# Aalto5G/pptk

Measured on AMD Instinct MI355X. Metric: Mpkts/s device-resident (cksum+parse+SipHash), 64B & 1500B; % HBM roofline, higher is better.
Workload: dtype u8

## Files before the change

### pptk_amd/csrc/rx_capi.hip

```cpp
#include <errno.h>
#include <stdlib.h>
#include <string.h>

#include <emmintrin.h>

#include <algorithm>
#include <atomic>
#include <condition_variable>
#include <memory>
#include <functional>
#include <mutex>
#include <new>
#include <thread>
#include <unordered_map>
#include <unordered_set>
#include <vector>

#include "../../include/hashseed.h"
#include "rx_internal.h"

using namespace pptk;

struct PartDesc {
  size_t bytes = 0, base = 0;
// ... 342 lines not shown
static int forced_variant(const pptk_rx_ctx *c) {
  static const long force = env_long("PPTK_RX_VARIANT", -1);
  if (c->forced_variant >= 0) return c->forced_variant;
  return force >= 0 && force < RX_NVARIANTS ? (int)force : -1;
}

static uint64_t resident_blocks(const pptk_rx_ctx *c, int variant);

static int grid_for(const pptk_rx_ctx *c, int variant, uint64_t n, uint32_t tpw = 0) {
  const uint64_t ntiles = (n + 63) / 64;
  const uint64_t want_blocks = (ntiles + kWavesPerBlock - 1) / kWavesPerBlock;
  if (tpw > 0) {
    const uint64_t per_block = (uint64_t)kWavesPerBlock * tpw;
    const uint64_t blocks = (ntiles + per_block - 1) / per_block;
    return (int)std::max<uint64_t>(1, std::min<uint64_t>(want_blocks,
                                                         std::max(blocks, resident_blocks(c, variant))));
  }
  return (int)std::max<uint64_t>(1, std::min<uint64_t>(want_blocks, resident_blocks(c, variant)));
}

static uint64_t resident_blocks(const pptk_rx_ctx *c, int variant) {
  static const long grid_mult = std::max(1l, EXP_KNOB("PPTK_RX_GRID_MULT", 1));
  static const int reserve_knob = (int)std::max(0l, EXP_KNOB("PPTK_RX_RESERVE_CUS", 0));
  const int reserve = std::max(reserve_knob, c->coll_cus);
  const uint64_t ncu = (uint64_t)std::max(1, c->ncu - std::min(reserve, c->ncu - 1));
  static const long bpc_knob = EXP_KNOB("PPTK_RX_BPC", 0);
  const uint64_t bpc = bpc_knob > 0 ? (uint64_t)bpc_knob : (uint64_t)c->bpc[variant];
  return ncu * bpc * (uint64_t)grid_mult;
}

static int plan_grid(const pptk_rx_ctx *c, int variant, uint64_t n, uint32_t tpw, RxKArgs &a);

static uint32_t tiles_per_wave(int variant, bool gather) {
  static const long lane = EXP_KNOB("PPTK_RX_LANE_TPW", 4);
  static const long strm = EXP_KNOB("PPTK_RX_GATHER_TPW", 8);
  static const long jumbo = EXP_KNOB("PPTK_RX_JUMBO_TPW", 0);
  static const long fixed = EXP_KNOB("PPTK_RX_FIXED_TPW", 0);
  if (variant == RX_L4) return (uint32_t)std::max(0l, lane);
  if (!gather) return (uint32_t)std::max(0l, fixed);
  return (uint32_t)std::max(0l, variant == RX_T64S2 ? jumbo : strm);
}

static int plan_grid(const pptk_rx_ctx *c, int variant, uint64_t n, uint32_t tpw, RxKArgs &a) {
  a.tail_block = 0;
  a.tail_tile = 0;
  const int grid = grid_for(c, variant, n, tpw);
  static const long pct = EXP_KNOB("PPTK_RX_TAIL_PCT", 0);
  static const long ttpw = EXP_KNOB("PPTK_RX_TAIL_TPW", 1);
  if (tpw == 0 || pct <= 0 || pct >= 100 || ttpw <= 0) return grid;
  const uint64_t ntiles = (n + 63) / 64;
  const uint64_t t2 = ntiles * (uint64_t)pct / 100, t1 = ntiles - t2;
  const uint64_t w1 = (uint64_t)kWavesPerBlock * tpw, w2 = (uint64_t)kWavesPerBlock * (uint64_t)ttpw;
  const uint64_t b1 = (t1 + w1 - 1) / w1, b2 = (t2 + w2 - 1) / w2;
  if (t2 == 0 || b1 < 2 * resident_blocks(c, variant) || b1 + b2 > 0x7fffffffull) return grid;
  a.tail_block = (uint32_t)b1;
  a.tail_tile = t1;
  return (int)(b1 + b2);
}

static uint64_t gcd64(uint64_t a, uint64_t b) {
  while (b) {
    const uint64_t t = a % b;
    a = b;
    b = t;
  }
  return a;
}

static int check_batch(const pptk_rx_ctx *c, const pptk_rx_dev_batch *b) {
  if (!c || !b) return -EINVAL;
  if (b->n == 0) return 0;
  if (!b->d_frames || (!b->d_recs && !b->d_recs32)) return -EINVAL;
  if (b->n > 0xffffffffull) return -EINVAL;
  if (!b->d_off && b->stride == 0 && b->n > 1) return -EINVAL;
  if (!b->d_len && b->fixed_len > 65535) return -EINVAL;
  return 0;
}

static RxKArgs batch_args(const pptk_rx_ctx *c, const pptk_rx_dev_batch *b) {
  RxKArgs a = c->tmpl;
  a.frames = b->d_frames;
  a.off = b->d_off;
  a.len = b->d_len;
  a.perm = b->d_perm;
  a.stride = b->stride;
  a.fixed_len = b->fixed_len;
  a.n = b->n;
  a.recs = b->d_recs;
  a.recs32 = b->d_recs32;
  a.hash = b->d_hash;
  a.frag = b->d_frag;
  a.key = b->d_key;
  return a;
}

static int auto_variant(const pptk_rx_dev_batch *b, bool *lane_ok_out) {
  uint32_t mmax = 15;
  if (!b->d_off) {
    const uint64_t p = (uint64_t)(uintptr_t)b->d_frames;
    const uint64_t gg = gcd64(b->stride % 16 ? b->stride % 16 : 16, 16);
    mmax = (uint32_t)((p % gg) + 16 - gg);
  }
  const uint32_t maxlen = b->d_len ? (b->max_len ? b->max_len : 65535u) : b->fixed_len;
  const bool lane_ok = !b->d_off && !b->d_len && !b->d_perm && !b->d_frag && mmax == 0 &&
                       b->fixed_len <= 64;
  if (lane_ok_out) *lane_ok_out = lane_ok;
  return lane_ok ? RX_L4 : pick_variant(maxlen + mmax);
}

static uint32_t phase_ticks_for(const pptk_rx_dev_batch *b, int variant, int grid) {
  static const long force = EXP_KNOB("PPTK_RX_PHASE_TICKS", -1);
  if (force >= 0) return (uint32_t)force;
  if (!rx_variant_phased(variant) || b->d_perm || (!b->d_recs && !b->d_recs32)) return 0;
  const uint64_t maxlen = b->d_len ? (b->max_len ? b->max_len : 1518u) : b->fixed_len;
  const uint64_t tile_bytes =
      64 * (b->d_off ? std::max<uint64_t>(64, maxlen / 2)
                     : std::min<uint64_t>(std::max<uint64_t>(b->stride, 64), 1u << 20));
  const uint64_t waves = (uint64_t)grid * kWavesPerBlock;
  const uint64_t ticks = tile_bytes * waves * 3 / 4 / 55000;
  return (uint32_t)std::min<uint64_t>(std::max<uint64_t>(ticks, 100), 1000000);
}

#ifdef PPTK_RX_WAVE_TIMES
static uint64_t *g_wave_times = nullptr;
static int g_wave_count = 0;
extern "C" int pptk_rx_wave_times(uint64_t *host, int max_waves) {
  if (!g_wave_times) return -EINVAL;
  const int n = std::min(max_waves, g_wave_count);
  if (hipDeviceSynchronize() != hipSuccess ||
      hipMemcpy(host, g_wave_times, (size_t)n * 16, hipMemcpyDeviceToHost) != hipSuccess)
    return -EIO;
  return n;
}
#endif

static int launch_batch(pptk_rx_ctx *c, const pptk_rx_dev_batch *b, int variant, void *stream) {
  RxKArgs a = batch_args(c, b);
  a.tune = pick_tune(c, variant, b->d_off || b->d_len || b->d_perm,
                     variant == RX_L4 && lane_coalesced(b->stride, b->fixed_len));
  c->last_variant = variant;
  const bool gather = b->d_off || b->d_len || b->d_perm;
  const int grid = plan_grid(c, variant, b->n, tiles_per_wave(variant, gather), a);
  a.phase_ticks = phase_ticks_for(
      b, variant, (int)std::min<uint64_t>((uint64_t)grid, resident_blocks(c, variant)));
#ifdef PPTK_RX_WAVE_TIMES
  if (!g_wave_times && hipMalloc(&g_wave_times, (size_t)65536 * 16) != hipSuccess) return -ENOMEM;
  if (grid * kWavesPerBlock > 65536) return -EINVAL;
  a.wave_times = g_wave_times;
  g_wave_count = grid * kWavesPerBlock;
#endif
  return hip_err(launch_rx(variant, a, grid, (hipStream_t)stream));
}

int pptk_rx_batch_device(struct pptk_rx_ctx *c, const struct pptk_rx_dev_batch *b,
                         void *stream) {
  int rc = check_batch(c, b);
  if (rc || b->n == 0) return rc;
  DeviceScope dg(c->device);
  if (!dg.ok) return -EIO;
  bool lane_ok = false;
  int variant = auto_variant(b, &lane_ok);
  const int tv = c->tuned[b->d_off || b->d_len || b->d_perm ? 1 : 0][variant];
  if (tv >= 0) variant = tv;
  const int fv = forced_variant(c);
  if (fv >= 0) variant = fv;
  if (variant == RX_L4 && !lane_ok) variant = auto_variant(b, nullptr);
  return launch_batch(c, b, variant, stream);
}

static int autotune_candidates(int variant, bool gather, int cand[8]) {
  int n = 0;
  cand[n++] = variant;
  if (variant == RX_T16S6) {
    cand[n++] = RX_T32S3;
    cand[n++] = RX_T32S3D7;
    cand[n++] = RX_T16S7L;
    if (gather) cand[n++] = RX_M6;
  }
  return n;
}

int pptk_rx_autotune(struct pptk_rx_ctx *c, const struct pptk_rx_dev_batch *b, int reps,
                     void *stream) {
  int rc = check_batch(c, b);
  if (rc || b->n == 0) return rc;
  if (reps < 1 || reps > 100) return -EINVAL;
  DeviceScope dg(c->device);
  if (!dg.ok) return -EIO;
  const int base = auto_variant(b, nullptr);
  const int g = b->d_off || b->d_len || b->d_perm ? 1 : 0;
  int cand[8];
  const int nc = autotune_candidates(base, g == 1, cand);
  hipEvent_t e0 = nullptr, e1 = nullptr;
  if (hipEventCreate(&e0) != hipSuccess || hipEventCreate(&e1) != hipSuccess) {
    (void)hipEventDestroy(e0);
    return -EIO;
  }
  const hipStream_t s = (hipStream_t)stream;
  std::vector<std::vector<float>> ms((size_t)nc);
  for (int r = 0; r < reps + 2 && rc == 0; ++r) {
    for (int k = 0; k < nc && rc == 0; ++k) {
      if (hipEventRecord(e0, s) != hipSuccess) rc = -EIO;
      if (rc == 0) rc = launch_batch(c, b, cand[k], stream);
      if (rc == 0 && (hipEventRecord(e1, s) != hipSuccess ||
                      hipEventSynchronize(e1) != hipSuccess))
        rc = -EIO;
      float t = 0.f;
      if (rc == 0 && r >= 2 && hipEventElapsedTime(&t, e0, e1) == hipSuccess)
        ms[(size_t)k].push_back(t);
    }
  }
  int best = base;
  if (rc == 0 && !ms[0].empty()) {
    std::vector<float> med((size_t)nc, 1e30f);
    for (int k = 0; k < nc; ++k) {
      if (ms[(size_t)k].empty()) continue;
      std::sort(ms[(size_t)k].begin(), ms[(size_t)k].end());
      med[(size_t)k] = ms[(size_t)k][ms[(size_t)k].size() / 2];
    }
    int kb = 0;
    for (int k = 1; k < nc; ++k)
      if (med[(size_t)k] < med[(size_t)kb]) kb = k;
    if (kb != 0 && med[(size_t)kb] < 0.99f * med[0]) best = cand[kb];
  }
  (void)hipEventDestroy(e0);
  (void)hipEventDestroy(e1);
  if (rc == 0) c->tuned[g][base] = best == base ? -1 : best;
  return rc;
}

int pptk_rx_place_buffers(struct pptk_rx_ctx *c, const struct pptk_rx_dev_batch *b,
                          const uint8_t *const *fr, int nf, void *const *rc_, int nr, int reps,
                          int *best_f, int *best_r, float *ms_out, void *stream) {
  if (!c || !b || !fr || !rc_ || !best_f || !best_r || nf < 1 || nf > 16 || nr < 1 ||
      nr > 64 || nf * nr > 256 || reps < 1 || reps > 100)
    return -EINVAL;
  for (int k = 0; k < nf; ++k)
    if (!fr[k]) return -EINVAL;
  for (int k = 0; k < nr; ++k)
    if (!rc_[k]) return -EINVAL;
  pptk_rx_dev_batch t = *b;
  const bool c32 = b->d_recs32 != nullptr;
  t.d_frames = fr[0];
  t.d_recs = c32 ? nullptr : (pptk_rx_rec *)rc_[0];
  t.d_recs32 = c32 ? (pptk_rx_rec32 *)rc_[0] : nullptr;
  int rc = check_batch(c, &t);
  if (rc || b->n == 0) {
    if (rc == 0) *best_f = *best_r = 0;
    return rc;
  }
  DeviceScope dg(c->device);
  if (!dg.ok) return -EIO;
  hipEvent_t e0 = nullptr, e1 = nullptr;
  if (hipEventCreate(&e0) != hipSuccess || hipEventCreate(&e1) != hipSuccess) {
    (void)hipEventDestroy(e0);
    return -EIO;
  }
  const hipStream_t s = (hipStream_t)stream;
  const int np = nf * nr;
  std::vector<std::vector<float>> ms((size_t)np);
  for (int r = 0; r <= reps && rc == 0; ++r) {
    for (int p = 0; p < np && rc == 0; ++p) {
      t.d_frames = fr[p / nr];
      if (c32) t.d_recs32 = (pptk_rx_rec32 *)rc_[p % nr];
      else t.d_recs = (pptk_rx_rec *)rc_[p % nr];
      if (hipEventRecord(e0, s) != hipSuccess) rc = -EIO;
      if (rc == 0) rc = pptk_rx_batch_device(c, &t, stream);
      if (rc == 0 && (hipEventRecord(e1, s) != hipSuccess || hipEventSynchronize(e1) != hipSuccess))
        rc = -EIO;
      float x = 0.f;
      if (rc == 0 && r > 0 && hipEventElapsedTime(&x, e0, e1) == hipSuccess)
        ms[(size_t)p].push_back(x);
    }
  }
  (void)hipEventDestroy(e0);
  (void)hipEventDestroy(e1);
  if (rc) return rc;
  int bp = 0;
  float bm = 1e30f;
  for (int p = 0; p < np; ++p) {
    std::vector<float> &v = ms[(size_t)p];
    std::sort(v.begin(), v.end());
    const float med = v.empty() ? 1e30f : v[v.size() / 2];
    if (ms_out) ms_out[p] = med;
    if (med < bm) {
      bm = med;
      bp = p;
    }
  }
  *best_f = bp / nr;
  *best_r = bp % nr;
  return 0;
}

int pptk_rx_place_records(struct pptk_rx_ctx *c, const struct pptk_rx_dev_batch *b,
                          void *const *cands, int ncand, int reps, int *best, float *ms_out,
                          void *stream) {
  if (!b || !best) return -EINVAL;
  const uint8_t *f0 = b->d_frames;
  int bf = 0;
  return pptk_rx_place_buffers(c, b, &f0, 1, cands, ncand, reps, &bf, best, ms_out, stream);
}

static bool tx_two_pass() {
  static const long v = EXP_KNOB("PPTK_TX_TWO_PASS", 1);
  return v != 0;
}

int pptk_tx_cksum_device(struct pptk_rx_ctx *c, uint8_t *d_frames, const uint64_t *d_off,
                         const uint16_t *d_len, uint64_t stride, uint32_t fixed_len,
                         uint64_t n, uint32_t max_len, void *stream) {
  if (!c || n > 0xffffffffull) return -EINVAL;
  if (n == 0) return 0;
  if (!d_frames || (!d_off && stride == 0 && n > 1) || (!d_len && fixed_len > 65535))
    return -EINVAL;
  DeviceScope dg(c->device);
  if (!dg.ok) return -EIO;
  pptk_rx_dev_batch b;
  memset(&b, 0, sizeof(b));
  b.d_frames = d_frames;
  b.d_off = d_off;
  b.d_len = d_len;
  b.stride = stride;
  b.fixed_len = fixed_len;
  b.max_len = max_len;
  b.n = n;
  uint32_t mmax = 15;
  if (!d_off) {
    const uint64_t p = (uint64_t)(uintptr_t)d_frames;
    const uint64_t gg = gcd64(stride % 16 ? stride % 16 : 16, 16);
    mmax = (uint32_t)((p % gg) + 16 - gg);
  }
  const uint32_t maxlen = d_len ? (max_len ? max_len : 65535u) : fixed_len;
  int variant = pick_variant(maxlen + mmax);
  const bool two_pass = !d_off && tx_two_pass();
  if (two_pass) {
    const int tv = c->tuned[0][variant];
    if (tv >= 0 && tv != RX_L4) variant = tv;
  }
  const int fv = forced_variant(c);
  if (fv >= 0 && fv != RX_L4) variant = fv;
  RxKArgs a = batch_args(c, &b);
  a.frames_w = d_frames;
  c->last_variant = variant;
  a.tune = c->forced_flags >= 0 ? (uint32_t)c->forced_flags & kTuneMask
                                : pick_tune(c, variant, d_off || d_len) &
                                      ~(uint32_t)PPTK_RX_TUNE_NT_LOADS;
  hipStream_t s = (hipStream_t)stream;
  if (two_pass) {
    if (c->forced_flags < 0)
      a.tune = pick_tune(c, variant, false);
    uint64_t *side = c->d_txuser && c->txuser_n >= n ? c->d_txuser : nullptr;
    const bool pooled = side == nullptr;
    if (pooled) {
      hipMemPool_t pool;
      {
        std::lock_guard<std::mutex> g(c->txpool_mu);
        if (!c->txpool) {
          hipMemPoolProps pp;
          memset(&pp, 0, sizeof(pp));
          pp.allocType = hipMemAllocationTypePinned;
          pp.location.type = hipMemLocationTypeDevice;
          pp.location.id = c->device;
          hipMemPool_t np = nullptr;
          if (hipMemPoolCreate(&np, &pp) != hipSuccess) return -ENOMEM;
          uint64_t keep = UINT64_MAX;
          (void)hipMemPoolSetAttribute(np, hipMemPoolAttrReleaseThreshold, &keep);
          c->txpool = np;
        }
        pool = c->txpool;
      }
      if (hipMallocFromPoolAsync((void **)&side, n * 8, pool, s) != hipSuccess)
        return -ENOMEM;
    }
    a.txside = side;
    hipError_t e = launch_rx(variant, a, grid_for(c, variant, n), s);
    if (e == hipSuccess) e = launch_tx_apply(side, d_frames, d_off, stride, n, s);
    if (pooled && hipFreeAsync(side, s) != hipSuccess && e == hipSuccess) e = hipErrorUnknown;
    return hip_err(e);
  }
  return hip_err(launch_rx(variant, a, grid_for(c, variant, n), s));
}

int pptk_tx_set_side_buffer(struct pptk_rx_ctx *c, void *d_side, uint64_t frames) {
  if (!c || (!d_side && frames) || ((uintptr_t)d_side & 7u)) return -EINVAL;
  DeviceScope dg(c->device);
  if (!dg.ok) return -EIO;
  c->d_txuser = (uint64_t *)d_side;
  c->txuser_n = d_side ? frames : 0;
  return 0;
}

int pptk_tx_rewrite_device(struct pptk_rx_ctx *c, uint8_t *d_frames, const uint64_t *d_off,
                           const uint16_t *d_len, uint64_t stride, uint32_t fixed_len,
                           uint64_t n, const struct pptk_rewrite *d_rw, uint64_t rw_count,
                           uint8_t *d_status, void *stream) {
  const bool ok = d_rw && (rw_count == 1 || rw_count == n);
  return hdr_op(c, d_frames, d_off, d_len, stride, fixed_len, n, d_status, ok,
                [&](const HdrBatch &b, int grid) {
                  const RewriteKArgs a = {b, d_rw, rw_count == 1 ? 1u : 0u};
                  return launch_rewrite(a, grid, (hipStream_t)stream);
                });
}

int pptk_tcp_mss_clamp_device(struct pptk_rx_ctx *c, uint8_t *d_frames, const uint64_t *d_off,
                              const uint16_t *d_len, uint64_t stride, uint32_t fixed_len,
                              uint64_t n, uint16_t mss, uint32_t flags, uint8_t *d_status,
                              void *stream) {
  const bool ok = !(flags & ~PPTK_MSS_SYN_ONLY);
  return hdr_op(c, d_frames, d_off, d_len, stride, fixed_len, n, d_status, ok,
                [&](const HdrBatch &b, int grid) {
                  const MssKArgs a = {b, mss, flags};
                  return launch_mss_clamp(a, grid, (hipStream_t)stream);
                });
}

int pptk_tcp_seq_translate_device(struct pptk_rx_ctx *c, uint8_t *d_frames, const uint64_t *d_off,
                                  const uint16_t *d_len, uint64_t stride, uint32_t fixed_len,
                                  uint64_t n, const struct pptk_seqxlate *d_xl, uint64_t xl_count,
                                  const uint32_t *d_idx, uint8_t *d_status, void *stream) {
  const bool ok = d_xl && xl_count != 0 && (d_idx || xl_count == 1 || xl_count == n);
  return hdr_op(c, d_frames, d_off, d_len, stride, fixed_len, n, d_status, ok,
                [&](const HdrBatch &b, int grid) {
                  const SeqKArgs a = {b, d_xl, xl_count, d_idx, !d_idx && xl_count == 1 ? 1u : 0u};
                  return launch_seq_translate(a, grid, (hipStream_t)stream);
                });
}

static const BinBounds &bin_bounds() {
  static const BinBounds bb = [] {
    BinBounds r;
    for (int k = 0; k < kGroups - 1; ++k) r.b[k] = kGroupMaxLen[k];
#ifdef PPTK_RX_EXPERIMENTS
    const char *e = getenv("PPTK_RX_BIN_BOUNDS");
#else
    const char *e = nullptr;
#endif
    if (!e) return r;
    BinBounds t = r;
    for (int k = 0; k < kGroups - 1; ++k) {
      char *end = nullptr;
      const unsigned long v = strtoul(e, &end, 10);
      if (end == e || v > 65535 || (k && v < t.b[k - 1])) return r;
      t.b[k] = (uint32_t)v;
      e = *end == ',' ? end + 1 : end;
    }
    return t;
  }();
  return bb;
}

static bool default_bounds(const BinBounds &bb) {
  for (int k = 0; k < kGroups - 1; ++k)
    if (bb.b[k] != kGroupMaxLen[k]) return false;
  return true;
}

int pptk_rx_batch_device_mixed(struct pptk_rx_ctx *c, const struct pptk_rx_dev_batch *b,
                               uint32_t *d_perm, void *d_scratch, void *stream) {
  int rc = check_batch(c, b);
  if (rc || b->n == 0) return rc;
  if (!b->d_len || !d_scratch) return -EINVAL;
  DeviceScope dg(c->device);
  if (!dg.ok) return -EIO;
  const hipStream_t s = (hipStream_t)stream;
  const BinBounds &bb = bin_bounds();
  const bool dflt = default_bounds(bb);
  if (b->max_len && b->max_len <= bb.b[kGroups - 2]) {
    pptk_rx_dev_batch t = *b;
    t.d_perm = nullptr;
    if ((rc = pptk_rx_batch_device(c, &t, stream)) != 0) return rc;
    return d_perm ? hip_err(launch_iota(d_perm, b->n, s)) : 0;
  }
  uint32_t *perm = d_perm ? d_perm : bin_perm(d_scratch, kBinGrid, b->n);
  BinDesc bd{b->d_off, b->stride, bin_desc_off(d_scratch, kBinGrid),
             bin_desc_len(d_scratch, kBinGrid, b->n)};
  hipError_t e = launch_bin(b->d_len, b->n, perm, d_scratch, s, kBinGrid, bd, bb, true);
  if (e != hipSuccess) return -EIO;
  RxKArgs a = batch_args(c, b);
  a.perm = perm;
  a.off = bd.boff;
  a.len = bd.blen;
  a.by_pos = 1;
  const uint32_t *tab = bin_table(d_scratch, kBinGrid);
  a.plan = tab + kGroups + 1;
  a.off0 = b->d_off;
  a.len0 = b->d_len;
  const uint32_t maxlen = b->max_len ? b->max_len : 65535u;
  const int fv = forced_variant(c);
  for (int g = 0; g < kGroups; ++g) {
    const bool last = g == kGroups - 1 || bb.b[g] >= maxlen;
    if (!last && g > 0 && bb.b[g] == bb.b[g - 1]) continue;
    int variant = fv >= 0 && fv != RX_L4 ? fv
                  : dflt || g == kGroups - 1 ? kGroupVariant[g]
                                             : pick_variant(bb.b[g] + 15);
    if (fv < 0 && c->tuned[1][variant] >= 0 && c->tuned[1][variant] != RX_L4)
      variant = c->tuned[1][variant];
    a.plan_group = (uint32_t)g;
    a.range_lo = tab + g;
    a.range_hi = tab + (last ? kGroups : g + 1);
    a.tune = pick_tune(c, variant, true);
    e = launch_rx(variant, a, grid_for(c, variant, b->n), s);
    if (e != hipSuccess) return -EIO;
    if (last) break;
  }
  return 0;
}

int pptk_rx_set_tuning(struct pptk_rx_ctx *c, int variant, int flags) {
  if (!c || variant < -1 || variant >= RX_NVARIANTS || flags < -1) return -EINVAL;
  if (flags >= 0 && ((uint32_t)flags & ~kTuneMask)) return -EINVAL;
  c->forced_variant = variant;
  const int rx = flags < 0 ? -1 : flags & ~PPTK_RX_TUNE_PERMIT_PASSES;
  c->forced_flags = flags >= 0 && rx == 0 && (flags & PPTK_RX_TUNE_PERMIT_PASSES) ? -1 : rx;
  c->permit_passes = flags >= 0 && (flags & PPTK_RX_TUNE_PERMIT_PASSES);
  return 0;
}

static constexpr int kSePerXcc = 4;

int pptk_rx_stream_split(struct pptk_rx_ctx *c, int coll_cus, void **rx_stream,
                         void **coll_stream) {
  if (!c || coll_cus < 0) return -EINVAL;
  if (coll_cus == 0) {
    if (rx_stream) *rx_stream = nullptr;
    if (coll_stream) *coll_stream = nullptr;
    c->coll_cus = 0;
    return 0;
  }
  if (!rx_stream || !coll_stream) return -EINVAL;
  *rx_stream = *coll_stream = nullptr;
  if (c->split_coll && c->split_cus == coll_cus) {
    *rx_stream = c->split_rx;
    *coll_stream = c->split_coll;
    c->coll_cus = coll_cus;
    return 0;
  }
  if (ctx_comm_slot(c)->load(std::memory_order_acquire) != nullptr) return -EBUSY;
  DeviceScope dg(c->device);
  if (!dg.ok) return -EIO;
  int nxcc = 1;
  if (hipDeviceGetAttribute(&nxcc, hipDeviceAttributeNumberOfXccs, c->device) != hipSuccess ||
      nxcc < 1)
    nxcc = 1;
  if (coll_cus % (nxcc * kSePerXcc) || coll_cus >= c->ncu || c->ncu % nxcc) return -EINVAL;
  std::vector<uint32_t> rx((c->ncu + 31) / 32, 0), coll(rx.size(), 0);
  for (int i = 0; i < c->ncu; ++i) (i >= c->ncu - coll_cus ? coll : rx)[i / 32] |= 1u << (i % 32);
  hipStream_t a = nullptr, b = nullptr;
  if (hipExtStreamCreateWithCUMask(&a, (uint32_t)rx.size(), rx.data()) != hipSuccess) return -EIO;
  if (hipExtStreamCreateWithCUMask(&b, (uint32_t)coll.size(), coll.data()) != hipSuccess) {
    (void)hipStreamDestroy(a);
    return -EIO;
  }
  drop_split_streams(c);
  {
    std::lock_guard<std::mutex> g(g_split_mu);
    g_split_owned[a] = c;
    g_split_owned[b] = c;
    g_split_retired.erase(a);
    g_split_retired.erase(b);
  }
  c->split_rx = a;
  c->split_coll = b;
  c->split_cus = coll_cus;
  *rx_stream = a;
  *coll_stream = b;
  c->coll_cus = coll_cus;
  return 0;
}

int pptk_rx_stream_destroy(void *stream) {
  if (!stream) return -EINVAL;
  const hipStream_t s = (hipStream_t)stream;
  {
    std::lock_guard<std::mutex> g(g_split_mu);
    if (g_split_owned.count(s)) return -EBUSY;
    if (g_split_retired.erase(s)) return 0;
  }
  return hip_err(hipStreamDestroy(s));
}

int pptk_rx_variant_count(void) { return RX_NVARIANTS; }

int pptk_rx_last_variant(const struct pptk_rx_ctx *c) { return c ? c->last_variant : -1; }

size_t pptk_rx_permit_scratch_bytes(uint64_t n, uint32_t hash_size) {
  if (hash_size == 0 || (hash_size & (hash_size - 1)) || n > 0xffffffffull) return 0;
  return permit_scratch_bytes(n, hash_size);
}

static int permit_common(struct pptk_rx_ctx *c, const struct pptk_rx_rec *d_recs,
                         const struct pptk_rx_rec32 *d_recs32, const uint32_t *d_keys,
                         uint64_t n, int family, const uint8_t *d_subject, uint32_t *d_tokens,
                         uint8_t *d_verdict, void *d_scratch, void *stream) {
  if (!c || (family != 4 && family != 6) || n > 0xffffffffull) return -EINVAL;
  if ((family == 4 && !c->opts.iphash_bits4) || (family == 6 && !c->opts.iphash_bits6))
    return -EINVAL;
  const uint32_t hs = c->opts.iphash_size;
  if (hs == 0 || (hs & (hs - 1))) return -EINVAL;
  if (n == 0) return 0;
  if ((!d_recs && !d_recs32 && !d_keys) || !d_tokens || !d_verdict || !d_scratch) return -EINVAL;
  DeviceScope dg(c->device);
  if (!dg.ok) return -EIO;
  PermitArgs a{};
  a.recs = d_recs32 || d_keys ? nullptr : d_recs;
  a.recs32 = d_keys ? nullptr : d_recs32;
  a.keys_in = d_keys;
  a.n = n;
  a.subject = d_subject;
  a.tokens = d_tokens;
  a.verdict = d_verdict;
  a.hash_size = hs;
  a.family = family;
  a.ncu = c->ncu - c->coll_cus;
  a.force_passes =
      c->permit_passes || (env_tune() >= 0 && (env_tune() & PPTK_RX_TUNE_PERMIT_PASSES)) ? 1 : 0;
  return hip_err(launch_permit(a, d_scratch, (hipStream_t)stream));
}

int pptk_rx_permit_status(struct pptk_rx_ctx *c, const void *d_scratch, void *stream) {
  if (!c || !d_scratch) return -EINVAL;
  DeviceScope dg(c->device);
  if (!dg.ok) return -EIO;
  return permit_status(d_scratch, (hipStream_t)stream);
}

int pptk_rx_permit_device(struct pptk_rx_ctx *c, const struct pptk_rx_rec *d_recs,
                          const struct pptk_rx_rec32 *d_recs32, uint64_t n, int family,
                          const uint8_t *d_subject, uint32_t *d_tokens, uint8_t *d_verdict,
                          void *d_scratch, void *stream) {
  if (!d_recs && !d_recs32) return -EINVAL;
  return permit_common(c, d_recs, d_recs32, nullptr, n, family, d_subject, d_tokens, d_verdict,
                       d_scratch, stream);
}

int pptk_rx_permit_keys_device(struct pptk_rx_ctx *c, const uint32_t *d_keys, uint64_t n,
                               int family, const uint8_t *d_subject, uint32_t *d_tokens,
                               uint8_t *d_verdict, void *d_scratch, void *stream) {
  if (!d_keys && n) return -EINVAL;
  return permit_common(c, nullptr, nullptr, d_keys, n, family, d_subject, d_tokens, d_verdict,
                       d_scratch, stream);
}

int pptk_rx_tokens_refill_device(struct pptk_rx_ctx *c, uint32_t *d_tokens, uint32_t start,
                                 uint32_t end, uint32_t add, uint32_t initial_tokens,
                                 void *stream) {
  if (!c || !d_tokens || start > end || end > c->opts.iphash_size) return -EINVAL;
  DeviceScope dg(c->device);
  if (!dg.ok) return -EIO;
  return hip_err(launch_refill(d_tokens, start, end, add, initial_tokens, (hipStream_t)stream));
}

size_t pptk_rx_bin_scratch_bytes(uint64_t n) { return bin_scratch_bytes(n, kBinGrid); }

// ... 464 lines not shown
```

### pptk_amd/csrc/rx_kernel.hip

```cpp
#include "frame_view.h"
#include "rx_internal.h"

#include <type_traits>

namespace pptk {

namespace {

constexpr int WAVE = 64;
constexpr int WPB = kWavesPerBlock;
constexpr int IMG_CHUNKS = 8;
#ifndef PPTK_RX_IMG_STRIDE
#define PPTK_RX_IMG_STRIDE 144
#endif
constexpr int IMG_STRIDE = PPTK_RX_IMG_STRIDE;
#ifndef PPTK_RX_TAIL_LDS
#define PPTK_RX_TAIL_LDS 1
#endif
constexpr bool TAIL_LDS = PPTK_RX_TAIL_LDS;
constexpr int TAIL_OFF = 128;
static_assert(!TAIL_LDS || (IMG_STRIDE >= TAIL_OFF + 16 && IMG_STRIDE % 16 == 0),
              "the parked tail chunk lives past the 128-byte image");

typedef uint64_t u64x2 __attribute__((ext_vector_type(2)));
// ... 496 lines not shown
    r1 = (u32x4){w[4], w[5], w[6], w[7]};
    r2 = (u32x4){w[8], w[9], w[10], w[11]};
    r3 = (u32x4){w[12], w[13], w[14], w[15]};
  }
  if (stage) {
    st[0] = r0; st[1] = r1;
    if (!c32) { st[2] = r2; st[3] = r3; }
  } else {
    GLB_AS u32x4 *dst = (GLB_AS u32x4 *)(c32 ? (GLB_AS uint8_t *)a.recs32 + (uint64_t)idx * 32u
                                             : (GLB_AS uint8_t *)a.recs + (uint64_t)idx * 64u);
    dst[0] = r0; dst[1] = r1;
    if (!c32) { dst[2] = r2; dst[3] = r3; }
  }
}

__device__ __forceinline__ void flush_records(const RxKArgs &a, const LDS_AS uint8_t *wimg, uint64_t tile,
                                              int lane, uint32_t my_idx, bool scatter,
                                              LDS_AS u32x4 *stash = nullptr) {
  const bool c32 = a.recs32 != nullptr;
  __builtin_amdgcn_wave_barrier();
  const LDS_AS u32x4 *st = (const LDS_AS u32x4 *)wimg;
  GLB_AS uint8_t *rbase = c32 ? (GLB_AS uint8_t *)a.recs32 : (GLB_AS uint8_t *)a.recs;
  GLB_AS u32x4 *dst = (GLB_AS u32x4 *)(rbase + tile * (uint64_t)WAVE * (c32 ? 32u : 64u));
  const uint64_t nrec = min((uint64_t)WAVE, a.n - tile * WAVE);
  const int lg = c32 ? 1 : 2;
  int kmax = c32 ? 2 : 4;
  if (kDiag && (a.tune & 128u)) kmax >>= 1;
#pragma unroll
  for (int k = 0; k < 4; ++k) {
    const int e = k * WAVE + lane;
    const int r = e >> lg;
    const int piece = e & ((1 << lg) - 1);
    GLB_AS u32x4 *d = dst + e;
    bool live = (uint64_t)r < nrec;
    if (scatter) {
      const uint32_t ridx = __shfl(my_idx, r & (WAVE - 1));
      live = ridx != 0xffffffffu;
      d = (GLB_AS u32x4 *)(rbase + (uint64_t)ridx * (c32 ? 32u : 64u)) + piece;
    }
    if (live && k < kmax) {
      const u32x4 val = st[r * 5 + piece];
      if (stash) {
        stash[e] = val;
      } else if (a.tune & 64u) {
        GLB_AS uint64_t *d8 = (GLB_AS uint64_t *)d;
        __hip_atomic_store(d8, (uint64_t)val.x | ((uint64_t)val.y << 32), __ATOMIC_RELAXED,
                           __HIP_MEMORY_SCOPE_AGENT);
        __hip_atomic_store(d8 + 1, (uint64_t)val.z | ((uint64_t)val.w << 32), __ATOMIC_RELAXED,
                           __HIP_MEMORY_SCOPE_AGENT);
      } else if (a.tune & 32u) {
        asm volatile("" ::: "memory");
        __builtin_nontemporal_store(val, d);
      } else {
        *d = val;
      }
    }
  }
  if (PPTK_RX_HASH_MODE == 2 && a.hash && !scatter && !a.perm && lane < WAVE / 2) {
    const uint32_t r0 = 2u * (uint32_t)lane;
    if ((uint64_t)r0 < nrec) {
      const uint64_t h0 = *(const LDS_AS uint64_t *)(st + r0 * 5 + 4);
      GLB_AS uint64_t *hd = (GLB_AS uint64_t *)a.hash + tile * (uint64_t)WAVE + r0;
      if ((uint64_t)r0 + 1 < nrec && ((uintptr_t)hd & 15u) == 0) {
        const uint64_t h1 = *(const LDS_AS uint64_t *)(st + (r0 + 1) * 5 + 4);
        const u64x2 v = {h0, h1};
        if (a.tune & 32u)
          __builtin_nontemporal_store(v, (GLB_AS u64x2 *)hd);
        else
          *(GLB_AS u64x2 *)hd = v;
      } else {
        hd[0] = h0;
        if ((uint64_t)r0 + 1 < nrec) hd[1] = *(const LDS_AS uint64_t *)(st + (r0 + 1) * 5 + 4);
      }
    }
  }
  __builtin_amdgcn_wave_barrier();
}

__device__ __forceinline__ uint64_t phase_deadline(uint32_t period) {
  const uint64_t rt = __builtin_amdgcn_s_memrealtime();
  return rt - rt % period + period;
}
__device__ __forceinline__ void flush_stash(const RxKArgs &a, const LDS_AS u32x4 *stash, uint64_t tile,
                                            int lane) {
  const bool c32 = a.recs32 != nullptr;
  GLB_AS uint8_t *rbase = c32 ? (GLB_AS uint8_t *)a.recs32 : (GLB_AS uint8_t *)a.recs;
  GLB_AS u32x4 *dst = (GLB_AS u32x4 *)(rbase + tile * (uint64_t)WAVE * (c32 ? 32u : 64u));
  const uint64_t nrec = min((uint64_t)WAVE, a.n - tile * WAVE);
  const int lg = c32 ? 1 : 2;
  const int kmax = c32 ? 2 : 4;
#pragma unroll
  for (int k = 0; k < 4; ++k) {
    const int e = k * WAVE + lane;
    if (k < kmax && (uint64_t)(e >> lg) < nrec) {
      const u32x4 val = stash[e];
      asm volatile("" ::: "memory");
      __builtin_nontemporal_store(val, dst + e);
    }
  }
}

struct TileRange {
  uint64_t first, step, end;
};
__device__ __forceinline__ TileRange wave_tiles(const RxKArgs &a, uint64_t ntiles, int wv) {
  const uint64_t wid = (uint64_t)blockIdx.x * WPB + wv;
  const uint64_t nwaves = (uint64_t)gridDim.x * WPB;
  if (a.tune & 256u) {
    const uint64_t per = (ntiles + nwaves - 1) / nwaves;
    return {wid * per, 1, min(ntiles, (wid + 1) * per)};
  }
  if (a.tail_block == 0) return {wid, nwaves, ntiles};
  if (blockIdx.x < a.tail_block) return {wid, (uint64_t)a.tail_block * WPB, min(a.tail_tile, ntiles)};
  return {a.tail_tile + (uint64_t)(blockIdx.x - a.tail_block) * WPB + wv,
          (uint64_t)(gridDim.x - a.tail_block) * WPB, ntiles};
}
__device__ __forceinline__ uint64_t pf_tile(const TileRange &r, uint64_t ntiles, uint64_t t) {
  return t < r.end ? t : ntiles;
}

template <int T, int S>
constexpr int min_waves_per_simd() { return S * T >= 32 ? 2 : 4; }
#ifndef PPTK_RX_D1_WAVES
#define PPTK_RX_D1_WAVES 3
#endif
template <int T, int S, int D>
constexpr int min_waves() { return D == 1 && S * T >= 32 ? PPTK_RX_D1_WAVES : min_waves_per_simd<T, S>(); }

__device__ __forceinline__ bool group_range(RxKArgs &a) {
  if (a.range_lo && a.plan && !(*a.plan & 1u)) {
    if (((*a.plan >> 8) & 0xffu) != a.plan_group) return false;
    a.perm = nullptr;
    a.perm_ld = (const uint32_t *)a.zero;
    a.perm_msk = 0u;
    a.off_ld = a.off0 ? a.off0 : (const uint64_t *)a.zero;
    a.off_msk = a.off0 ? ~0u : 0u;
    a.stride_g = a.off0 ? 0u : a.stride;
    a.len_ld = a.len0;
    a.len_msk = ~0u;
    a.by_pos = 0;
  } else if (a.range_lo) {
    const uint32_t lo = *a.range_lo, hi = *a.range_hi;
    a.perm_ld += lo;
    if (a.by_pos) {
      a.off_ld += lo;
      a.len_ld += lo;
    }
    a.n = hi > lo ? hi - lo : 0;
    if (a.n == 0) return false;
  }
  return true;
}

template <int T, int S, int D, int AL, bool NT, bool GATHER>
__global__ __launch_bounds__(WAVE * WPB, (min_waves<T, S, D>())) void rx_kernel(RxKArgs a) {
  if constexpr (GATHER) {
    if (!group_range(a)) return;
  }
  __shared__ __attribute__((aligned(16))) uint8_t lds[WPB * WAVE * IMG_STRIDE];
  constexpr int IMGC = (S * T < IMG_CHUNKS) ? S * T : IMG_CHUNKS;
  constexpr uint32_t ALM = (1u << AL) - 1;
  static_assert(T % (D + 1) == 0, "prefetch ring must wrap at the tile boundary");
  constexpr bool PHASED = S * T >= 32 && T <= 32;
  __shared__ __attribute__((aligned(16))) u32x4 stash_lds[PHASED ? WPB * 4 * WAVE : 1];
  const bool phased = PHASED && a.phase_ticks != 0;
  uint64_t st_tile = ~0ull;
  uint64_t st_deadline = 0;
  constexpr bool UNROLL = T <= 32;
  const int lane = threadIdx.x & (WAVE - 1);
  const int wv = threadIdx.x / WAVE;
  const int g = lane / T, j = lane % T;
  LDS_AS uint8_t *wimg = (LDS_AS uint8_t *)lds + wv * WAVE * IMG_STRIDE;
  LDS_AS u32x4 *stash = (LDS_AS u32x4 *)stash_lds + (PHASED ? wv * 4 * WAVE : 0);
  const uint64_t ntiles = (a.n + WAVE - 1) / WAVE;
  const TileRange tr = wave_tiles(a, ntiles, wv);
  const uint64_t step = tr.step, tend = tr.end;

  uint64_t tile = tr.first;
#ifdef PPTK_RX_WAVE_TIMES
  const uint64_t wid = (uint64_t)blockIdx.x * WPB + wv;
  const uint64_t wt_start = __builtin_amdgcn_s_memrealtime();
#endif
  Desc dc = load_desc<GATHER>(a, pf_tile(tr, ntiles, tile), lane);
  Desc dn = load_desc<GATHER>(a, pf_tile(tr, ntiles, tile + step), lane);
  uint32_t idx2 = desc_idx<GATHER>(a, pf_tile(tr, ntiles, tile + 2 * step), lane);
  Buf<S> b[D + 1];
#pragma unroll
  for (int k = 0; k < D; ++k) {
    b[k] = load_round<T, S, AL, NT>(a, dc, k, g, j);
    __builtin_amdgcn_sched_barrier(0);
  }

  while (tile < tend) {
    uint32_t my_sum = 0;
    const uint32_t idx3 = desc_idx<GATHER>(a, pf_tile(tr, ntiles, tile + 3 * step), lane);
    auto group = [&](const int r0) __attribute__((always_inline)) {
#pragma unroll
      for (int u = 0; u <= D; ++u) {
        const int r = r0 + u;
        {
          const int rr = r + D;
          const Desc &dd = rr < T ? dc : dn;
          b[(u + D) % (D + 1)] = load_round<T, S, AL, NT>(a, dd, rr < T ? rr : rr - T, g, j);
        }
        const Buf<S> &cb = b[u];
        const int q = g * T + r;
        const int m = (int)(cb.pb & ALM);
        const int c_img = m >> 4;
        const int nch = (m + (int)cb.pl + 15) >> 4;
        LDS_AS uint8_t *img = wimg + q * IMG_STRIDE;
#pragma unroll
        for (int s = 0; s < S; ++s) {
          if (s * T < IMGC + (int)(ALM >> 4)) {
            const int ci = s * T + j - c_img;
            if (ci >= 0 && ci < IMGC) {
              if constexpr (IMG_STRIDE % 16 == 0) {
                *(LDS_AS u32x4 *)(img + 16 * ci) = cb.v[s];
              } else {
                LDS_AS uint32_t *w = (LDS_AS uint32_t *)(img + 16 * ci);
                w[0] = cb.v[s].x;
                w[1] = cb.v[s].y;
                w[2] = cb.v[s].z;
                w[3] = cb.v[s].w;
              }
            }
          }
        }
        uint32_t acc = 0;
        const int ts = team_start_of(m & 15);
#pragma unroll
        for (int s = 0; s < S; ++s) {
          const int c = s * T + j;
          acc = sum_chunk_from<!GATHER>(cb.v[s], 16 * c - m, ts, (int)cb.pl, acc);
        }
        if (!UNROLL && nch > S * T) {
          const u32x4 *c0 = (const u32x4 *)(a.frames + (cb.pb - (uint64_t)m));
          for (int c = S * T + j; c < nch; c += T)
            acc = sum_chunk_from<true>(ldc<NT>(c0 + c), 16 * c - m, ts, (int)cb.pl, acc);
        }
        if constexpr (GATHER) {
          if constexpr (TAIL_LDS) {
            if (j == T - 1) *(LDS_AS u32x4 *)(img + TAIL_OFF) = cb.v[S - 1];
          } else {
            const uint32_t corr = tail_past_end(cb.v[S - 1], m, (int)cb.pl, ts);
            acc -= (j == T - 1 && nch <= S * T) ? corr : 0u;
          }
        }
        acc = team_sum<T>(acc);
        if (j == r)
          my_sum = acc;
        if (PHASED && u < D && st_tile != ~0ull && __builtin_amdgcn_s_memrealtime() >= st_deadline) {
          flush_stash(a, stash, st_tile, lane);
          st_tile = ~0ull;
        }
      }
    };
#ifdef PPTK_RX_FULL_UNROLL
#pragma unroll(T <= 16 ? T : 1)
#else
#pragma unroll 1
#endif
    for (int r0 = 0; r0 < T - (D + 1); r0 += D + 1) {
      group(r0);
      if (PHASED && st_tile != ~0ull && __builtin_amdgcn_s_memrealtime() >= st_deadline) {
        flush_stash(a, stash, st_tile, lane);
        st_tile = ~0ull;
      }
    }
    const Desc d2 = desc_fill<GATHER>(a, idx2, pf_tile(tr, ntiles, tile + 2 * step), lane);
    __builtin_amdgcn_sched_barrier(0);
    group(T - (D + 1));

    const bool stage = !(a.tune & 2u);
    const bool scatter = GATHER && a.perm;
    if (dc.idx != 0xffffffffu && !(kDiag && (a.tune & 16u))) {
      const int m = (int)(dc.base & 15);
      const int ma = (int)(dc.base & ALM);
      const int nch = (ma + (int)dc.len + 15) >> 4;
      u32x4 tailc = (u32x4){0u, 0u, 0u, 0u};
      if constexpr (GATHER && TAIL_LDS) {
        const u32x4 t = *(const LDS_AS u32x4 *)(wimg + lane * IMG_STRIDE + TAIL_OFF);
        const bool fits = nch <= S * T;
        tailc = (u32x4){fits ? t.x : 0u, fits ? t.y : 0u, fits ? t.z : 0u, fits ? t.w : 0u};
      }
      if (UNROLL) {
        if (nch > S * T) {
          const u32x4 *c0 = (const u32x4 *)(a.frames + (dc.base - (uint64_t)ma));
          for (int c = S * T; c < nch; ++c)
            my_sum = settle(sum_chunk_from<true>(ldc<NT>(c0 + c), 16 * c - ma, 0, (int)dc.len,
                                                 my_sum));
        }
      }
      const FrameView v = {wimg + lane * IMG_STRIDE, (const GLB_AS uint8_t *)a.frames + dc.base, m,
                           16 * IMGC - m};
      LaneRec o;
      lane_generic(a, v, dc.len, dc.base, my_sum, tailc, o);
      if (a.txside)
        a.txside[dc.idx] = o.tx;
      emit_record(a, o, dc.idx, (LDS_AS u32x4 *)wimg + lane * 5, stage);
    }
    if (stage && !(kDiag && (a.tune & 8u)) && (a.recs || a.recs32)) {
      if (PHASED && phased && !scatter) {
        if (st_tile != ~0ull) flush_stash(a, stash, st_tile, lane);
        flush_records(a, wimg, tile, lane, dc.idx, scatter, stash);
        st_tile = tile;
        st_deadline = phase_deadline(a.phase_ticks);
      } else {
        flush_records(a, wimg, tile, lane, dc.idx, scatter);
      }
    }
    tile += step;
    dc = dn;
    dn = d2;
    idx2 = idx3;
  }
  if (PHASED && st_tile != ~0ull) flush_stash(a, stash, st_tile, lane);
#ifdef PPTK_RX_WAVE_TIMES
  if (a.wave_times && lane == 0) {
    a.wave_times[2 * wid] = wt_start;
    a.wave_times[2 * wid + 1] = __builtin_amdgcn_s_memrealtime();
  }
#endif
}

constexpr int M_S = 6;
#ifndef PPTK_RX_M_D
#define PPTK_RX_M_D 1
#endif
#ifndef PPTK_RX_M_WAVES
#define PPTK_RX_M_WAVES 3
#endif
constexpr int M_D = PPTK_RX_M_D;
constexpr int M_SUM = 128;
static_assert(IMG_STRIDE >= M_SUM + 4, "the team sum lives past the 128-byte image");

struct MSched {
  uint32_t n0, n1, n2, e0, e1, e2;
};

__device__ __forceinline__ uint32_t m_rank(uint64_t mask) {
  return __builtin_amdgcn_mbcnt_hi((uint32_t)(mask >> 32),
                                   __builtin_amdgcn_mbcnt_lo((uint32_t)mask, 0u));
}

constexpr int M_RMAX = 24;
__device__ __forceinline__ MSched m_schedule(const Desc &d, int lane, LDS_AS uint8_t *list) {
  const bool valid = d.idx != 0xffffffffu;
  const uint32_t nch = ((uint32_t)(d.base & 15u) + d.len + 15u) >> 4;
  const uint64_t b0 = __ballot(valid && nch <= 24u);
  const uint64_t b1 = __ballot(valid && nch > 24u && nch <= 48u);
  const uint64_t b2 = __ballot(valid && nch > 48u);
  MSched s;
  s.n0 = (uint32_t)__popcll(b0);
  s.n1 = (uint32_t)__popcll(b1);
  s.n2 = (uint32_t)__popcll(b2);
  s.e0 = (s.n0 + 15u) >> 4;
  s.e1 = s.e0 + ((s.n1 + 7u) >> 3);
  s.e2 = s.e1 + ((s.n2 + 3u) >> 2);
  LDS_AS uint32_t *lw = (LDS_AS uint32_t *)list;
  lw[lane] = 0xffffffffu;
  if (lane < M_RMAX * 4 - WAVE) lw[WAVE + lane] = 0xffffffffu;
  const uint32_t c = nch <= 24u ? 0u : nch <= 48u ? 1u : 2u;
  const uint32_t rho = c == 0u ? m_rank(b0) : c == 1u ? m_rank(b1) : m_rank(b2);
  const uint32_t er = c == 0u ? 0u : c == 1u ? s.e0 : s.e1;
  const uint32_t sh = 4u - c;
  if (valid) list[(er + (rho >> sh)) * 16u + (rho & ((1u << sh) - 1u))] = (uint8_t)lane;
  return s;
}

__device__ __forceinline__ uint32_t m_rounds(const MSched &s) {
  constexpr uint32_t G = M_D + 1;
  return s.e2 <= 2 * G ? 2 * G : (s.e2 + G - 1) / G * G;
}

__device__ __forceinline__ int m_tl(const MSched &s, uint32_t r) {
  return r < s.e0 ? 2 : r < s.e1 ? 3 : 4;
}

template <int CTRL>
__device__ __forceinline__ uint32_t m_dpp(uint32_t x) {
  return (uint32_t)__builtin_amdgcn_update_dpp(0, (int)x, CTRL, 0xf, 0xf, true);
}
__device__ __forceinline__ uint32_t m_team_sum(uint32_t x, int tl) {
  x += m_dpp<0xb1>(x);
  x += m_dpp<0x4e>(x);
  const uint32_t x8 = x + m_dpp<0x114>(x);
  x = tl >= 3 ? x8 : x;
  const uint32_t x16 = x + m_dpp<0x118>(x);
  return tl >= 4 ? x16 : x;
}

struct MBuf {
  u32x4 v[M_S];
  uint32_t qml;
};

template <bool NT>
__device__ __forceinline__ MBuf m_load_round(const RxKArgs &a, const Desc &d, const MSched &s,
                                             const LDS_AS uint8_t *list, uint32_t r, int lane) {
  const int tl = m_tl(s, r);
  const uint32_t e = list[r * 16u + ((uint32_t)lane >> tl)];
  const bool real = e != 0xffu;
  const uint32_t q = e & (WAVE - 1);
  MBuf b;
  const uint64_t pb = __shfl(d.base, (int)q);
  const uint32_t pl = __shfl(d.len, (int)q) & (0u - (uint32_t)real);
  const int m = (int)(pb & 15u);
  b.qml = (real ? q : 0xffu) | ((uint32_t)m << 8) | (pl << 16);
  const u32x4 *c0 = (const u32x4 *)(a.frames + (pb - (uint64_t)m));
  const int nch = (m + (int)pl + 15) >> 4;
  const int clast = nch > 0 ? nch - 1 : 0;
  const int j = lane & ((1 << tl) - 1);
#pragma unroll
  for (int i = 0; i < M_S; ++i)
    b.v[i] = ldc<NT>(c0 + min((i << tl) + j, clast));
  return b;
}

template <bool NT, bool GATHER>
__global__ __launch_bounds__(WAVE * WPB, PPTK_RX_M_WAVES) void rx_kernel_mixed(RxKArgs a) {
  if constexpr (GATHER) {
    if (!group_range(a)) return;
  }
  __shared__ __attribute__((aligned(16))) uint8_t lds[WPB * WAVE * IMG_STRIDE];
  __shared__ __attribute__((aligned(16))) uint8_t lists[WPB][2][M_RMAX * 16];
  const int lane = threadIdx.x & (WAVE - 1);
  const int wv = threadIdx.x / WAVE;
  LDS_AS uint8_t *wimg = (LDS_AS uint8_t *)lds + wv * WAVE * IMG_STRIDE;
  LDS_AS uint8_t *lst[2] = {(LDS_AS uint8_t *)lists[wv][0], (LDS_AS uint8_t *)lists[wv][1]};
  const uint64_t ntiles = (a.n + WAVE - 1) / WAVE;
  const TileRange tr = wave_tiles(a, ntiles, wv);
  const uint64_t step = tr.step, tend = tr.end;

  uint64_t tile = tr.first;
  Desc dc = load_desc<GATHER>(a, pf_tile(tr, ntiles, tile), lane);
  Desc dn = load_desc<GATHER>(a, pf_tile(tr, ntiles, tile + step), lane);
  uint32_t idx2 = desc_idx<GATHER>(a, pf_tile(tr, ntiles, tile + 2 * step), lane);
  int cur = 0;
// ... 325 lines not shown
```

Measured before the change: 4258.

## Cooperatively checksum oversized frame tails across the wave and retune gather variant choice

Frames whose length exceeds the tile's staged chunks used to be checksummed by each owning lane serially. A wave-cooperative loop now handles them instead: every lane loads one 16-byte chunk of the current overflow frame, with a K-deep software-pipelined prefetch, and the partial sums are reduced with a team sum back to the owner lane. Separately, untuned gather batches on the T64S2 shape now default to T16S7L, and the mixed-size path skips binning when tuning picked a 1536-shape variant. This trades per-lane divergence on long frames for extra register pressure and wave-level reduction overhead.

Result: no change. 4226 (-0.8%).

```diff
diff --git a/pptk_amd/csrc/rx_capi.hip b/pptk_amd/csrc/rx_capi.hip
--- a/pptk_amd/csrc/rx_capi.hip
+++ b/pptk_amd/csrc/rx_capi.hip
@@ -518,6 +518,8 @@
   return hip_err(launch_rx(variant, a, grid, (hipStream_t)stream));
 }
 
+static int untuned_shape(int variant, bool gather);
+
 int pptk_rx_batch_device(struct pptk_rx_ctx *c, const struct pptk_rx_dev_batch *b,
                          void *stream) {
   int rc = check_batch(c, b);
@@ -526,8 +528,9 @@
   if (!dg.ok) return -EIO;
   bool lane_ok = false;
   int variant = auto_variant(b, &lane_ok);
-  const int tv = c->tuned[b->d_off || b->d_len || b->d_perm ? 1 : 0][variant];
-  if (tv >= 0) variant = tv;
+  const bool gather = b->d_off || b->d_len || b->d_perm;
+  const int tv = c->tuned[gather ? 1 : 0][variant];
+  variant = tv >= 0 ? tv : untuned_shape(variant, gather);
   const int fv = forced_variant(c);
   if (fv >= 0) variant = fv;
   if (variant == RX_L4 && !lane_ok) variant = auto_variant(b, nullptr);
@@ -536,6 +539,13 @@
 
 static int autotune_candidates(int variant, bool gather, int cand[8]) {
   int n = 0;
+  if (variant == RX_T64S2 && gather) {
+    cand[n++] = RX_T16S7L;
+    cand[n++] = RX_T16S6;
+    cand[n++] = RX_T32S3;
+    cand[n++] = RX_T64S2;
+    return n;
+  }
   cand[n++] = variant;
   if (variant == RX_T16S6) {
     cand[n++] = RX_T32S3;
@@ -544,6 +554,17 @@
     if (gather) cand[n++] = RX_M6;
   }
   return n;
+}
+
+static int untuned_shape(int variant, bool gather) {
+  int cand[8];
+  (void)autotune_candidates(variant, gather, cand);
+  return cand[0];
+}
+
+static bool shape_1536(int variant) {
+  return variant == RX_T16S6 || variant == RX_T16S7L || variant == RX_T32S3 ||
+         variant == RX_T32S3D7 || variant == RX_T16S6D1;
 }
 
 int pptk_rx_autotune(struct pptk_rx_ctx *c, const struct pptk_rx_dev_batch *b, int reps,
@@ -576,7 +597,7 @@
         ms[(size_t)k].push_back(t);
     }
   }
-  int best = base;
+  int best = cand[0];
   if (rc == 0 && !ms[0].empty()) {
     std::vector<float> med((size_t)nc, 1e30f);
     for (int k = 0; k < nc; ++k) {
@@ -591,7 +612,7 @@
   }
   (void)hipEventDestroy(e0);
   (void)hipEventDestroy(e1);
-  if (rc == 0) c->tuned[g][base] = best == base ? -1 : best;
+  if (rc == 0) c->tuned[g][base] = best == base && cand[0] == base ? -1 : best;
   return rc;
 }
 
@@ -832,7 +853,9 @@
   const hipStream_t s = (hipStream_t)stream;
   const BinBounds &bb = bin_bounds();
   const bool dflt = default_bounds(bb);
-  if (b->max_len && b->max_len <= bb.b[kGroups - 2]) {
+  const int fv = forced_variant(c);
+  const bool tuned_1536 = fv < 0 && shape_1536(c->tuned[1][RX_T64S2]);
+  if ((b->max_len && b->max_len <= bb.b[kGroups - 2]) || tuned_1536) {
     pptk_rx_dev_batch t = *b;
     t.d_perm = nullptr;
     if ((rc = pptk_rx_batch_device(c, &t, stream)) != 0) return rc;
@@ -853,7 +876,6 @@
   a.off0 = b->d_off;
   a.len0 = b->d_len;
   const uint32_t maxlen = b->max_len ? b->max_len : 65535u;
-  const int fv = forced_variant(c);
   for (int g = 0; g < kGroups; ++g) {
     const bool last = g == kGroups - 1 || bb.b[g] >= maxlen;
     if (!last && g > 0 && bb.b[g] == bb.b[g - 1]) continue;
@@ -866,6 +888,7 @@
     a.range_lo = tab + g;
     a.range_hi = tab + (last ? kGroups : g + 1);
     a.tune = pick_tune(c, variant, true);
+    c->last_variant = variant;
     e = launch_rx(variant, a, grid_for(c, variant, b->n), s);
     if (e != hipSuccess) return -EIO;
     if (last) break;
diff --git a/pptk_amd/csrc/rx_kernel.hip b/pptk_amd/csrc/rx_kernel.hip
--- a/pptk_amd/csrc/rx_kernel.hip
+++ b/pptk_amd/csrc/rx_kernel.hip
@@ -672,6 +672,95 @@
   return true;
 }
 
+struct OvCur {
+  uint64_t mask;
+  const u32x4 *c0;
+  int ma, len, nch;
+  int c;
+  int q;
+};
+
+__device__ __forceinline__ uint32_t bcast_lane(uint32_t x, int q) {
+  return (uint32_t)__builtin_amdgcn_readlane((int)x, q);
+}
+
+template <int FIT, uint32_t ALM>
+__device__ __forceinline__ void ov_open(OvCur &cu, const RxKArgs &a, const Desc &d) {
+  cu.q = __builtin_ctzll(cu.mask);
+  const uint64_t base = (uint64_t)bcast_lane((uint32_t)d.base, cu.q) |
+                        ((uint64_t)bcast_lane((uint32_t)(d.base >> 32), cu.q) << 32);
+  cu.len = (int)bcast_lane(d.len, cu.q);
+  cu.ma = (int)(base & ALM);
+  cu.c0 = (const u32x4 *)(a.frames + (base - (uint64_t)cu.ma));
+  cu.nch = (cu.ma + cu.len + 15) >> 4;
+  cu.c = FIT;
+}
+
+template <int FIT, uint32_t ALM>
+__device__ __forceinline__ void ov_next(OvCur &cu, const RxKArgs &a, const Desc &d) {
+  if (cu.c < cu.nch) {
+    cu.c += WAVE;
+    if (cu.c >= cu.nch && (cu.mask & (cu.mask - 1))) {
+      cu.mask &= cu.mask - 1;
+      ov_open<FIT, ALM>(cu, a, d);
+    }
+  }
+}
+
+template <bool NT>
+__device__ __forceinline__ u32x4 ov_load(const OvCur &cu, int lane) {
+  return ldc<NT>(cu.c0 + min(cu.c + lane, cu.nch - 1));
+}
+
+__device__ __forceinline__ void ov_sum(const OvCur &cu, u32x4 v, int lane, uint32_t &acc,
+                                       uint32_t &my_sum) {
+  acc = sum_chunk_from<true>(v, 16 * (cu.c + lane) - cu.ma, 0, cu.len, acc);
+  if (cu.c < cu.nch && cu.c + WAVE >= cu.nch) {
+    const uint32_t tot = team_sum<WAVE>(acc);
+    my_sum += lane == cu.q ? tot : 0u;
+    acc = 0;
+  }
+}
+
+template <int T, int S, int D>
+constexpr int ov_steps() { return min_waves<T, S, D>() > 2 || D > 3 ? 4 : 8; }
+
+template <int T, int S, int D, uint32_t ALM, bool NT>
+__device__ __forceinline__ void ov_tile(const RxKArgs &a, const Desc &d, int lane,
+                                        uint32_t &my_sum) {
+  constexpr int K = ov_steps<T, S, D>();
+  const int nch = ((int)(d.base & ALM) + (int)d.len + 15) >> 4;
+  const uint64_t over = __ballot(d.idx != 0xffffffffu && nch > S * T);
+  if (over == 0) return;
+  OvCur ld, su;
+  ld.mask = over;
+  ov_open<S * T, ALM>(ld, a, d);
+  su = ld;
+  u32x4 v[K];
+#pragma unroll
+  for (int k = 0; k < K; ++k) {
+    v[k] = ov_load<NT>(ld, lane);
+    ov_next<S * T, ALM>(ld, a, d);
+  }
+  uint32_t acc = 0;
+  while (ld.c < ld.nch) {
+#pragma unroll
+    for (int k = 0; k < K; ++k) {
+      ov_sum(su, v[k], lane, acc, my_sum);
+      ov_next<S * T, ALM>(su, a, d);
+      v[k] = ov_load<NT>(ld, lane);
+      ov_next<S * T, ALM>(ld, a, d);
+    }
+  }
+#pragma unroll
+  for (int k = 0; k < K; ++k) {
+    ov_sum(su, v[k], lane, acc, my_sum);
+    ov_next<S * T, ALM>(su, a, d);
+    acc = settle(acc);
+  }
+  my_sum = settle(my_sum);
+}
+
 template <int T, int S, int D, int AL, bool NT, bool GATHER>
 __global__ __launch_bounds__(WAVE * WPB, (min_waves<T, S, D>())) void rx_kernel(RxKArgs a) {
   if constexpr (GATHER) {
@@ -687,6 +776,7 @@
   uint64_t st_tile = ~0ull;
   uint64_t st_deadline = 0;
   constexpr bool UNROLL = T <= 32;
+  constexpr bool OVSUM = UNROLL && GATHER && S * T >= 96;
   const int lane = threadIdx.x & (WAVE - 1);
   const int wv = threadIdx.x / WAVE;
   const int g = lane / T, j = lane % T;
@@ -790,6 +880,7 @@
     const Desc d2 = desc_fill<GATHER>(a, idx2, pf_tile(tr, ntiles, tile + 2 * step), lane);
     __builtin_amdgcn_sched_barrier(0);
     group(T - (D + 1));
+    if constexpr (OVSUM) ov_tile<T, S, D, ALM, NT>(a, dc, lane, my_sum);
 
     const bool stage = !(a.tune & 2u);
     const bool scatter = GATHER && a.perm;
@@ -803,7 +894,7 @@
         const bool fits = nch <= S * T;
         tailc = (u32x4){fits ? t.x : 0u, fits ? t.y : 0u, fits ? t.z : 0u, fits ? t.w : 0u};
       }
-      if (UNROLL) {
+      if (UNROLL && !OVSUM) {
         if (nch > S * T) {
           const u32x4 *c0 = (const u32x4 *)(a.frames + (dc.base - (uint64_t)ma));
           for (int c = S * T; c < nch; ++c)
```
